# GoekeLab/m6anet

Hardware: AMD Instinct MI355X
Metric: DRACH sites/sec at num_iterations=1000 (higher is better)
Workload: dtype f32

## Files before the change

m6anet_amd/csrc/m6a_api.hip:

```cpp
#include "m6a_ctx.h"

#if !defined(__HIP_DEVICE_COMPILE__)
#ifndef M6A_MT_JUMP_PATH
#error "build with -DM6A_MT_JUMP_PATH=\"<repo>/m6anet_amd/assets/mt19937_jump.bin\" (m6anet_amd/build.py does)"
#endif
asm(".section .rodata\n"
    ".global m6a_mt_jump_blob\n.global m6a_mt_jump_blob_end\n.hidden m6a_mt_jump_blob\n.hidden m6a_mt_jump_blob_end\n.balign 64\n"
    "m6a_mt_jump_blob:\n.incbin \"" M6A_MT_JUMP_PATH "\"\n"
    "m6a_mt_jump_blob_end:\n.byte 0\n.previous\n");
#endif

namespace {

thread_local std::string g_create_error;

std::mutex g_live_mu;
std::vector<m6a_ctx *> g_live;
void join_background_setups()
{
    std::lock_guard<std::mutex> g(g_live_mu);
    for (m6a_ctx *c : g_live)
        if (c->warm.joinable()) c->warm.join();
    g_live.clear();
}
// ... 527 lines not shown
    c->bag_min = (int64_t)c->h_minmax[0];
    c->bag_max = (int64_t)c->h_minmax[1];
    c->n_reads = (int64_t)c->h_minmax[2];
    return M6A_OK;
}

int bag_stats(m6a_ctx *c, const int64_t *d_off, int64_t S)
{
    const int64_t *h = c->hint_off;
    c->hint_off = nullptr;
    if (!h) return query_bags(c, d_off, S);
    if (h[0] != 0) return fail(c, M6A_EINVAL, "off[0] must be 0");
    host_bag_range(c, h, S);
    if (c->bag_min < 0) return fail(c, M6A_EINVAL, "off[] must be non-decreasing");
    unsigned long long hash = 0;
    for (int i = 0; i < M6A_HIST_BINS; i++) hash += (unsigned long long)c->h_hist[i] * m6a_bin_weight(i);
    hipStream_t st = c->s_prep ? c->s_prep : c->stream;
    if (st != c->stream) {
        HIPCHK(c, hipEventRecord(c->ev_main, c->stream));
        HIPCHK(c, hipStreamWaitEvent(st, c->ev_main, 0));
    }
    HIPCHK(c, hipMemsetAsync(c->d_minmax, 0xff, 8, st));
    HIPCHK(c, hipMemsetAsync(c->d_minmax + 1, 0, 16, st));
    HIPCHK(c, hipMemsetAsync(c->d_hist, 0, M6A_HIST_BINS * 4, st));
    hipLaunchKernelGGL(bag_minmax_kernel, dim3((unsigned)std::min<int64_t>((S + 255) / 256, 512)), dim3(256), 0,
                       st, d_off, S, c->d_minmax, c->d_hist);
    hipLaunchKernelGGL(bag_verify_kernel, dim3(1), dim3(256), 0, st, c->d_minmax, c->d_hist, (unsigned long long)c->bag_min,
                       (unsigned long long)c->bag_max, (unsigned long long)c->n_reads, hash, c->d_err);
    HIPCHK(c, hipGetLastError());
    c->side_work = true;
    return M6A_OK;
}

static unsigned enc_args(m6a_ctx *c, EncArgs &a, const float *X, const uint8_t *km, const int64_t *off, int64_t S, int64_t R, float *rp)
{
    a.X = X; a.site_kmers = km; a.off = off; a.wfrag = c->d_wfrag; a.emb = c->d_emb; a.read_prob = rp;
    a.wfrag2 = c->d_wfrag2; a.w1e_tab = c->d_w1e; a.bn = c->d_w1e + M6A_W1E_FLOATS; a.err = c->d_err;
    a.n_sites = S; a.n_reads = R; a.n_tiles = (R + 31) / 32; a.b3 = c->b3;
    a.clk = nullptr;
    const int64_t max_waves = (int64_t)c->n_cu * 8;
    a.tiles_per_wave = (a.n_tiles + max_waves - 1) / max_waves;
    const int64_t waves = (a.n_tiles + a.tiles_per_wave - 1) / a.tiles_per_wave;
    return (unsigned)((waves + 3) / 4);
}

int launch_encode(m6a_ctx *c, const float *X, const uint8_t *km, const int64_t *off, int64_t S,
                  int64_t R, float *rp)
{
    if (R <= 0 || S <= 0) return M6A_OK;
    EncArgs a;
    const unsigned blocks = enc_args(c, a, X, km, off, S, R, rp);
    a.clk = c->prof.clk_for(0);
    const bool fits32 = S < 0x7ffffff0LL && a.n_tiles < 0x7ffffff0LL;
    if (c->enc_variant == 2 && !fits32) return fail(c, M6A_EUNSUPPORTED, "12-slot encoder: more than 2^31 sites or tiles");
    const bool scalar_chain = c->bag_min >= M6A_CSITE_MIN_BAG && fits32;
    const bool csite = c->enc_variant == 2 || (c->enc_variant == 4 && scalar_chain);
    const bool site16 = !csite && c->enc_variant != 3 && scalar_chain;
    c->enc_variant_used = csite ? "csite12" : "general16";
    c->enc_kernel_used = csite ? "enc_csite_kernel" : site16 ? "enc_site16_kernel" : "enc_kernel";
    prof_begin(c, 0);
    if (csite) hipLaunchKernelGGL(enc_csite_kernel, dim3(blocks), dim3(256), 0, c->stream, a);
    else if (site16) hipLaunchKernelGGL(enc_site16_kernel, dim3(blocks), dim3(256), 0, c->stream, a);
    else hipLaunchKernelGGL(enc_kernel, dim3(blocks), dim3(256), 0, c->stream, a);
    prof_end(c, 0);
    HIPCHK(c, hipGetLastError());
    return M6A_OK;
}

int launch_repr(m6a_ctx *c, const float *X, const uint8_t *km, const int64_t *off, int64_t S, int64_t R, void *repr, int dtype, float *rp)
{
    if (R <= 0 || S <= 0) return M6A_OK;
    EncReprArgs ra;
    const unsigned blocks = enc_args(c, ra.enc, X, km, off, S, R, rp);
    ra.repr = repr;
    c->enc_variant_used = "general16";
    c->enc_kernel_used = dtype == M6A_REPR_F16 ? "enc_repr_kernel<true>" : "enc_repr_kernel";
    prof_begin(c, 0);
    if (dtype == M6A_REPR_F16)
        hipLaunchKernelGGL(enc_repr_kernel<true>, dim3(blocks), dim3(256), 0, c->stream, ra);
    else
        hipLaunchKernelGGL(enc_repr_kernel<false>, dim3(blocks), dim3(256), 0, c->stream, ra);
    prof_end(c, 0);
    HIPCHK(c, hipGetLastError());
    return M6A_OK;
}

int repr_writer_begin(m6a_ctx *c, int device, hipStream_t *stream)
{
    settle(c);
    HintScope hint_scope(c);
    if (c->job.open) return job_busy(c);
    if (c->device != device) return fail(c, M6A_EINVAL, "the context is on device %d, the sites are on device %d", c->device, device);
    HIPCHK(c, hipSetDevice(c->device));
    *stream = c->stream;
    return M6A_OK;
}

int repr_writer_round(m6a_ctx *c, const float *X, const uint8_t *km, const int64_t *off, int64_t *off_round, int64_t s0, int64_t s1,
                      int64_t r0, int64_t nr, void *repr, int dtype)
{
    if (nr <= 0 || s1 <= s0) return M6A_OK;
    hipLaunchKernelGGL(rebase_off_kernel, dim3((unsigned)((s1 - s0 + 1 + 255) / 256)), dim3(256), 0, c->stream, off + s0, s1 - s0 + 1, off_round);
    HIPCHK(c, hipGetLastError());
    return launch_repr(c, X + r0 * 9, km + s0 * 3, off_round, s1 - s0, nr, repr, dtype, nullptr);
}

RtabUse rtab_use(m6a_ctx *c, int64_t nmax, uint32_t si_base = 0, uint32_t si_count = 0)
{
    RtabUse u;
    u.C = c->rt.C; u.RS = c->rt.RS; u.slot_of_n = (const int32_t *)c->ctl_dev.p + M6A_HIST_BINS;
    u.rank = (uint32_t *)c->rt_rank.p; u.order = (const uint32_t *)c->rt_order.p;
    u.c_stride = c->rt.n_blk * 64; u.n_blk = (uint32_t)c->rt.n_blk;
    u.bag_cap = (int)std::max<int64_t>(64, (nmax + 63) / 64 * 64);
    u.si_base = si_base; u.si_count = si_count;
    return u;
}

int rtab_prepare(m6a_ctx *c, hipStream_t st, PoolArgs a, int64_t nmax, int64_t gmax, uint32_t seed, bool *use)
{
    *use = false;
    const int T = a.T, K = a.K;
    const int64_t S = a.n_sites;
    const int64_t need = stream_need(gmax, T, K);
    if (nmax > M6A_RTAB_MAX_N || c->scan_driver == 1 || c->scan_driver == 2) {
        if (c->scan_driver == 3)
            return fail(c, M6A_EUNSUPPORTED, "index-table pooling needs every bag <= %d reads (largest: %lld)", M6A_RTAB_MAX_N, (long long)nmax);
        return M6A_OK;
    }
    int distinct = 0;
    const int missing = rtab_missing(c, seed, T, K, need, c->h_hist, &distinct);
    if (c->rt_credit_seed != seed || c->rt_credit_A != (int64_t)T * K) { c->rt_credit_seed = seed; c->rt_credit_A = (int64_t)T * K; c->rt_credit = 0; }
    bool use_rtab = c->scan_driver == 3 || missing == 0 || c->rt_credit + S >= (int64_t)16 * missing;
    if (use_rtab) c->rt_credit = 0; else c->rt_credit += S;
    if (!use_rtab) return M6A_OK;
    int rc = ensure_rtab(c, st, seed, T, K, gmax, c->h_hist, &use_rtab);
    if (rc) return rc;
    if (!use_rtab) return M6A_OK;
// ... 27 lines not shown
    unsigned blocks = 0, start_blocks = 0;
    size_t lds = 0;
    int64_t n_big = 0, cap_big = 0, cap_small = 0;
};

int pool_plan(m6a_ctx *c, hipStream_t st, const int64_t *off, int64_t S, int T, int K, uint32_t seed, int64_t bs, int64_t spb,
              PoolPlan *p)
{
    *p = PoolPlan();
    PoolArgs &a = p->a;
    if (S <= 0) return M6A_OK;
    if (c->site_mode == M6A_SITE_EXPECTED) {
        if (!base_is_group_start(c->job_offset, bs, spb))
            return fail(c, M6A_EINVAL, "job offset %lld does not start a flush group for batch_size=%lld save_per_batch=%lld",
                        (long long)c->job_offset, (long long)bs, (long long)spb);
        if (c->bag_min < 0 || c->bag_max > 0x7fffffff) return fail(c, M6A_EINVAL, "off[] is not a non-decreasing CSR array");
        a.off = off; a.n_sites = S; a.K = K;
        p->bag_min = c->bag_min; p->bag_max = c->bag_max;
        p->kind = PoolPlan::expected;
        return M6A_OK;
    }
    int rc = ensure_groups(c, st, S, bs, spb);
    if (rc) return rc;
    const int64_t nmin = c->bag_min, nmax = c->bag_max;
    if (nmin < 0 || nmax > 0x7fffffff) return fail(c, M6A_EINVAL, "off[] is not a non-decreasing CSR array");
    a.off = off; a.goff = (const int64_t *)c->goff.p; a.err = c->d_err;
    a.n_groups = c->goff_key.G; a.n_sites = S; a.T = T; a.K = K;
    const int64_t gmax = c->goff_key.gmax;

    rc = ensure_mean_plan(c, st, T);
    if (rc) return rc;
    plan_args(c, a);
    const bool uniform = nmin == nmax && nmin >= 1 && nmin <= M6A_TABLE_MAX_N && K == 20 && gmax <= 4096;
    const bool reg_ok = uniform && c->plan.depth <= M6A_REG_STACK && c->n_reads < (int64_t)1 << 30 &&
                        (int64_t)gmax * (T + 8) * K * 2 <= (int64_t)256 << 20;
    if (uniform && reg_ok && c->table_variant != 1) {
        rc = ensure_table_reg(c, st, seed, (int)nmin, T, K, (int)gmax);
        if (rc) return rc;
        a.tab = (const uint32_t *)c->tab_reg.p; a.uniform_n = (int)nmin; a.jmax = (int)gmax;
        const int64_t wpj = (a.n_groups + 255) / 256;
        a.reg_items = wpj * a.jmax;
        p->blocks = (unsigned)((a.reg_items + 7) / 8 * 8);
        p->kind = PoolPlan::table_reg;
        return M6A_OK;
    }
    if (uniform && c->plan.max_merge <= 15) {
        rc = ensure_table(c, st, seed, (int)nmin, T, K, (int)gmax);
        if (rc) return rc;
        a.tab = (const uint32_t *)c->tab.p; a.uniform_n = (int)nmin; a.jmax = (int)gmax;
        const int64_t gblocks = (a.n_groups + 7) / 8;
        int64_t nbj = std::max<int64_t>(1, ((int64_t)c->n_cu * 5 + a.jmax - 1) / a.jmax);
        nbj = std::min<int64_t>(nbj, (gblocks + 3) / 4);
        p->blocks = (unsigned)(nbj * a.jmax);
        p->lds = (size_t)4 * (128 + 8 * a.stack_depth) * sizeof(float);
        p->kind = PoolPlan::table;
        return M6A_OK;
    }
    bool use_rtab = false;
    rc = rtab_prepare(c, st, a, nmax, gmax, seed, &use_rtab);
    if (rc) return rc;
    if (use_rtab) {
        a.raw = (const uint32_t *)c->raw.p; a.raw_len = c->raw_len;
        for (int n = M6A_RTAB_SMALL_N + 1; n < M6A_HIST_BINS; n++) p->n_big += c->h_hist[n];
        p->cap_big = nmax; p->cap_small = std::min<int64_t>(nmax, M6A_RTAB_SMALL_N);
        p->kind = PoolPlan::ragged_table;
        return M6A_OK;
    }
// ... 492 lines not shown
        rc = bag_stats(c, off, S);
        if (rc) return rc;
        return launch_repr(c, X, km, off, S, c->n_reads, repr, dtype, rp);
    }
    rc = csr_check(c, off, S);
    if (rc) return rc;
    const int64_t R = off[S];
    if (R == 0) return M6A_OK;
    const int64_t chunk_reads = (int64_t)1 << 20;
    std::vector<int64_t> cs{0};
    int64_t widest = 0;
    while (cs.back() < S) {
        const int64_t s0 = cs.back();
        int64_t s1 = std::upper_bound(off + s0, off + S + 1, off[s0] + chunk_reads) - off - 1;
        s1 = std::min<int64_t>(S, std::max<int64_t>(s1, s0 + 1));
        widest = std::max(widest, off[s1] - off[s0]);
        cs.push_back(s1);
    }
    const int64_t nchunk = (int64_t)cs.size() - 1;
    HIPCHK(c, c->sX.ensure((size_t)widest * 9 * 4));
    HIPCHK(c, c->sOffChunk.ensure((size_t)(S + nchunk) * 8));
    HIPCHK(c, c->sRepr.ensure((size_t)widest * row_bytes));
    if (rp) HIPCHK(c, c->sP.ensure((size_t)widest * 4));
    HIPCHK(c, stage_in(c, c->sK, km, (size_t)S * 3));
    HIPCHK(c, stage_in(c, c->sOff, off, (size_t)(S + 1) * 8));
    for (int64_t k = 0; k < nchunk; k++) {
        const int64_t s0 = cs[k], s1 = cs[k + 1], r0 = off[s0], nr = off[s1] - r0;
        if (nr == 0) continue;
        HIPCHK(c, hipMemcpyAsync(c->sX.p, X + r0 * 9, (size_t)nr * 9 * 4, hipMemcpyHostToDevice, c->stream));
        int64_t *d_off = (int64_t *)c->sOffChunk.p + s0 + k;
        hipLaunchKernelGGL(rebase_off_kernel, dim3((unsigned)((s1 - s0 + 1 + 255) / 256)), dim3(256), 0, c->stream,
                           (const int64_t *)c->sOff.p + s0, s1 - s0 + 1, d_off);
        rc = launch_repr(c, (const float *)c->sX.p, (const uint8_t *)c->sK.p + s0 * 3, d_off, s1 - s0, nr, c->sRepr.p, dtype,
                         rp ? (float *)c->sP.p : nullptr);
        if (rc) return rc;
        HIPCHK(c, stage_out(c, (char *)repr + (size_t)r0 * row_bytes, c->sRepr, (size_t)nr * row_bytes));
        if (rp) HIPCHK(c, stage_out(c, rp + r0, c->sP, (size_t)nr * 4));
        HIPCHK(c, hipStreamSynchronize(c->stream));
    }
    return sync_and_check(c);
}

static int pool_stage_in(m6a_ctx *c, const float *rp, const int64_t *off, int64_t S, bool sigma)
{
    int rc = csr_check(c, off, S);
    if (rc) return rc;
    HIPCHK(c, c->sSite.ensure((size_t)S * 4));
    HIPCHK(c, c->sMod.ensure((size_t)S * 8));
    if (sigma) HIPCHK(c, c->sSigma.ensure((size_t)S * 8));
    HIPCHK(c, stage_in(c, c->sP, rp, (size_t)off[S] * 4));
    HIPCHK(c, stage_in(c, c->sOff, off, (size_t)(S + 1) * 8));
    host_bag_range(c, off, S);
    return M6A_OK;
}

static int pool_stage_out(m6a_ctx *c, int64_t S, float *site, double *mod, double *sigma)
{
    HIPCHK(c, stage_out(c, site, c->sSite, (size_t)S * 4));
    HIPCHK(c, stage_out(c, mod, c->sMod, (size_t)S * 8));
    if (sigma) HIPCHK(c, stage_out(c, sigma, c->sSigma, (size_t)S * 8));
    return sync_and_check(c);
}

int m6a_site_pool(m6a_ctx *c, const float *rp, const int64_t *off, int64_t S, int T, int K, float thr,
                  uint32_t seed, int rng_mode, int64_t bs, int64_t spb, float *site, double *mod)
{
    HintScope hint_scope(c);
// ... 279 lines not shown
```

m6anet_amd/csrc/m6a_ctx.h:

```cpp
#pragma once
#include <hip/hip_runtime.h>
#include <dlfcn.h>
#include <sys/mman.h>

#include <algorithm>
#include <atomic>
#include <cmath>
#include <cstdarg>
#include <cstdio>
#include <cstdlib>
#include <cstring>
#include <condition_variable>
#include <functional>
#include <memory>
#include <mutex>
#include <new>
#include <string>
#include <thread>
#include <vector>

#include "m6a.h"
#include "m6a_kernels.h"
#include "m6a_host_cpus.h"

// ... 256 lines not shown

static inline int enter(m6a_ctx *c)
{
    settle(c);
    if (!c) return M6A_EINVAL;
    return job_busy(c);
}

static inline int same_side(m6a_ctx *c, const void *first, std::initializer_list<const void *> rest, const char *sentence)
{
    const bool dev = is_device_ptr(first);
    for (const void *p : rest)
        if (p && dev != is_device_ptr(p)) return fail(c, M6A_EINVAL, "%s", sentence);
    return dev;
}

static inline int csr_check(m6a_ctx *c, const int64_t *off, int64_t S)
{
    if (off[0] != 0) return fail(c, M6A_EINVAL, "off[0] must be 0");
    for (int64_t s = 0; s < S; s++) if (off[s + 1] < off[s]) return fail(c, M6A_EINVAL, "off[] must be non-decreasing");
    return M6A_OK;
}

static inline hipError_t stage_in(m6a_ctx *c, DevBuf &b, const void *host, size_t bytes)
{
    const hipError_t e = b.ensure(bytes ? bytes : 1);
    return e != hipSuccess ? e : hipMemcpyAsync(b.p, host, bytes, hipMemcpyHostToDevice, c->stream);
}
static inline hipError_t stage_out(m6a_ctx *c, void *host, const DevBuf &b, size_t bytes)
{
    return hipMemcpyAsync(host, b.p, bytes, hipMemcpyDeviceToHost, c->stream);
}

int launch_encode(m6a_ctx *c, const float *X, const uint8_t *km, const int64_t *off, int64_t S, int64_t R, float *rp);
int launch_repr(m6a_ctx *c, const float *X, const uint8_t *km, const int64_t *off, int64_t S, int64_t R, void *repr, int dtype, float *rp);
int repr_writer_begin(m6a_ctx *c, int device, hipStream_t *stream);
int repr_writer_round(m6a_ctx *c, const float *X, const uint8_t *km, const int64_t *off, int64_t *off_round, int64_t s0, int64_t s1,
                      int64_t r0, int64_t nr, void *repr, int dtype);
int launch_pool(m6a_ctx *c, const float *rp, const int64_t *off, int64_t S, int T, int K, float thr, uint32_t seed, int64_t bs, int64_t spb,
                float *site, double *mod);
int bag_stats(m6a_ctx *c, const int64_t *d_off, int64_t S);
void host_bag_range(m6a_ctx *c, const int64_t *off, int64_t S);
void prof_begin(m6a_ctx *c, int kind);
void prof_end(m6a_ctx *c, int kind);
int ensure_staging(m6a_ctx *c);
void release_staging(m6a_ctx *c);
int staged_encode(m6a_ctx *c, const float *X, const uint8_t *km, const int64_t *off, int64_t S, int64_t R, float *rp_host);
int staged_outputs(m6a_ctx *c, int64_t S, float *site, double *mod);
int d2h_through_ring(m6a_ctx *c, void *host, const void *dev, size_t bytes);
bool base_is_group_start(int64_t base, int64_t bs, int64_t spb);
void comm_release(m6a_ctx *c);

}
```

m6anet_amd/csrc/m6a_job.hip:

```cpp
#include "m6a_ctx.h"

using namespace m6a_detail;

namespace m6a_detail {

int grow_keep(m6a_ctx *c, DevBuf &b, size_t used_bytes, size_t need_bytes)
{
    if (need_bytes <= b.cap) return M6A_OK;
    const size_t want = std::max(need_bytes + need_bytes / 8 + 256, b.cap * 2);
    void *np_ = nullptr;
    HIPCHK(c, hipMalloc(&np_, want));
    if (b.p && used_bytes) {
        if (c->stg.s_h2d) HIPCHK(c, hipStreamSynchronize(c->stg.s_h2d));
        HIPCHK(c, hipMemcpyAsync(np_, b.p, used_bytes, hipMemcpyDeviceToDevice, c->stream));
        HIPCHK(c, hipStreamSynchronize(c->stream));
    }
    if (b.p) (void)hipFree(b.p);
    b.p = np_; b.cap = want;
    return M6A_OK;
}

int job_setup_ring(m6a_ctx *c)
{
    auto &j = c->job;
// ... 36 lines not shown
    if (!j.cur_ready) {
        if (j.used[(size_t)sub]) HIPCHK(c, hipEventSynchronize(j.ev_h2d[(size_t)sub]));
        j.cur_ready = true;
    }
    *pin = j.pin[(size_t)sub];
    return M6A_OK;
}

int job_flush(m6a_ctx *c, const float *dX = nullptr, const uint8_t *dK = nullptr)
{
    auto &j = c->job;
    Staging &g = c->stg;
    if (j.fill_sites == 0) return M6A_OK;
    const int sub = (int)(j.item % j.n_sub);
    char *pin = j.pin[(size_t)sub];
    char *dev = (char *)c->jX.p + (size_t)sub * j.sub_bytes;
    const int64_t ns = j.fill_sites, nr = j.fill_reads, s0 = j.S - ns, r0 = j.R - nr;
    int rc = grow_keep(c, c->jP, (size_t)r0 * 4, (size_t)std::max<int64_t>(j.R, 1) * 4);
    if (rc) return rc;
    rc = grow_keep(c, c->jOff, (size_t)(s0 + 1) * 8, (size_t)(j.S + 1) * 8);
    if (rc) return rc;
    if (j.used[(size_t)sub]) HIPCHK(c, hipStreamWaitEvent(g.s_h2d, j.ev_enc[(size_t)sub], 0));
    HIPCHK(c, hipMemcpyAsync(dev, pin, (size_t)(ns + 1) * 8, hipMemcpyHostToDevice, g.s_h2d));
    HIPCHK(c, hipMemcpyAsync((int64_t *)c->jOff.p + s0, pin + j.o_goff, (size_t)(ns + 1) * 8, hipMemcpyHostToDevice, g.s_h2d));
    if (!dX) {
        HIPCHK(c, hipMemcpyAsync(dev + j.o_km, pin + j.o_km, (size_t)ns * 3, hipMemcpyHostToDevice, g.s_h2d));
        if (nr) HIPCHK(c, hipMemcpyAsync(dev + j.o_x, pin + j.o_x, (size_t)nr * M6A_N_FEATURES * 4, hipMemcpyHostToDevice, g.s_h2d));
    }
    HIPCHK(c, hipEventRecord(j.ev_h2d[(size_t)sub], g.s_h2d));
    HIPCHK(c, hipStreamWaitEvent(c->stream, j.ev_h2d[(size_t)sub], 0));
    if (nr) {
        c->bag_min = j.fill_min; c->n_reads = nr;
        rc = launch_encode(c, dX ? dX : (const float *)(dev + j.o_x), dK ? dK : (const uint8_t *)(dev + j.o_km), (const int64_t *)dev, ns, nr,
                           (float *)c->jP.p + r0);
        if (rc) return rc;
    }
    HIPCHK(c, hipEventRecord(j.ev_enc[(size_t)sub], c->stream));
    j.used[(size_t)sub] = 1;
    j.item++; j.chunks++;
    j.fill_sites = 0; j.fill_reads = 0; j.fill_min = INT64_MAX; j.cur_ready = false;
    return M6A_OK;
}

void job_append_offsets(m6a_ctx *c, char *pin, const int64_t *off, int64_t i, int64_t k)
{
    auto &j = c->job;
    int64_t *ol = (int64_t *)pin, *og = (int64_t *)(pin + j.o_goff);
    if (j.fill_sites == 0) { ol[0] = 0; og[0] = j.R; }
    const int64_t base = off[i], lbase = j.fill_reads, gbase = j.R;
    int64_t mn = j.fill_min;
    for (int64_t t = 0; t < k; t++) {
        const int64_t e = off[i + t + 1] - base, n = off[i + t + 1] - off[i + t];
        ol[j.fill_sites + t + 1] = lbase + e;
        og[j.fill_sites + t + 1] = gbase + e;
        j.off.push_back(gbase + e);
        mn = n < mn ? n : mn;
    }
    j.fill_min = mn;
    const int64_t nr = off[i + k] - base;
    j.fill_sites += k; j.fill_reads += nr; j.S += k; j.R += nr;
}

int job_feed_impl(m6a_ctx *c, const float *X, const uint8_t *km, const int64_t *off, int64_t n, bool dev)
{
    auto &j = c->job;
    int rc = csr_check(c, off, n);
    if (rc) return rc;
// ... 213 lines not shown
```

m6anet_amd/csrc/m6a_kernels.h:

```cpp
#ifndef M6A_KERNELS_H
#define M6A_KERNELS_H
#include <hip/hip_runtime.h>
#include <stdint.h>

#define M6A_BAG_LDS 1024
#define M6A_WFRAG_FLOATS (136 * 64)
#define M6A_WFRAG2_FLOATS (25 * 64)
#define M6A_W1E_FLOATS (35 * 32)
#define M6A_BN_FLOATS (5 * 2 * 16 * 2)
#define M6A_MEAN_STACK 32
#define M6A_CSITE_MIN_BAG 16
#define M6A_TABLE_MAX_N 32
#define M6A_REG_STACK 8
#define M6A_RTAB_MAX_N 4096
#define M6A_RTAB_SMALL_N 1024
#define M6A_RTAB_U8_MAX_N 256
#define M6A_HIST_BINS (M6A_RTAB_MAX_N + 2)

__host__ __device__ inline unsigned long long m6a_bin_weight(int i)
{
    unsigned long long z = (unsigned long long)(i + 1) * 0x9E3779B97F4A7C15ull;
    z = (z ^ (z >> 30)) * 0xBF58476D1CE4E5B9ull;
    z = (z ^ (z >> 27)) * 0x94D049BB133111EBull;
    return z ^ (z >> 31);
}

#define M6A_CLK_SLOTS 64
__device__ __forceinline__ void m6a_clk_stamp(unsigned long long *clk, int which)
{
    if (!clk) return;
    const unsigned stride = (gridDim.x >> 6) | 1u, b = blockIdx.x;
    if (threadIdx.x == 0 && b % stride == 0 && b / stride < M6A_CLK_SLOTS) {
        unsigned long long *p = clk + (size_t)(b / stride) * 4 + which * 2;
        p[0] = __builtin_amdgcn_s_memtime();
        p[1] = __builtin_amdgcn_s_memrealtime();
    }
}

struct EncArgs {
    const float *X;
    const uint8_t *site_kmers;
    const int64_t *off;
    const float *wfrag;
    const float *wfrag2;
    const float *w1e_tab;
    const float *bn;
    const float *emb;
    float *read_prob;
    int *err;
    int64_t n_sites, n_reads, n_tiles, tiles_per_wave;
    float b3;
    unsigned long long *clk;
};

struct EncReprArgs {
    EncArgs enc;
    void *repr;
};

struct PoolArgs {
    const float *read_prob;
    const int64_t *off;
    const int64_t *goff;
    const uint32_t *raw;
    const uint32_t *tab;
    float *site_prob;
    double *mod_ratio;
    uint32_t *start_pos;
    const int *leaf_start;
    const uint8_t *merge_after;
    const uint32_t *row_meta;
    int n_leaves, n_rows, n_rem;
    int stack_depth;
    const uint32_t *reg_ctl;
    int reg_rounds, reg_final_merges;
    int64_t reg_items;
    int *err;
    int64_t n_groups, n_sites, raw_len;
    int T, K, uniform_n, jmax, bag_cap;
    float thr;
    unsigned long long *clk;
};

// ... 70 lines not shown
```

m6anet_amd/csrc/m6a_kernels.hip:

```cpp
#include <hip/hip_runtime.h>
#include <stdint.h>

#include "m6a_kernels.h"

typedef float f32x16 __attribute__((ext_vector_type(16)));
typedef float f32x2 __attribute__((ext_vector_type(2)));

__device__ __forceinline__ float chain8_sum(float r)
{
    r += __builtin_bit_cast(float, __builtin_amdgcn_update_dpp(0, __builtin_bit_cast(int, r), 0xB1, 0xf, 0xf, false));
    r += __builtin_bit_cast(float, __builtin_amdgcn_update_dpp(0, __builtin_bit_cast(int, r), 0x4E, 0xf, 0xf, false));
    r += __builtin_bit_cast(float, __builtin_amdgcn_update_dpp(0, __builtin_bit_cast(int, r), 0x141, 0xf, 0xf, false));
    return r;
}

__device__ __forceinline__ int wave_sum_i32(int v)
{
#pragma unroll
    for (int m = 1; m < 64; m <<= 1) v += __shfl_xor(v, m, 64);
    return v;
}

#define L2_REGS(m) ((m) == 4 ? 12 : 16)

// ... 99 lines not shown
{
    return ((int64_t)__builtin_amdgcn_readfirstlane((int)(v >> 32)) << 32) |
           (uint32_t)__builtin_amdgcn_readfirstlane((int)v);
}

__device__ __forceinline__ void wave_lds_fence()
{
    __builtin_amdgcn_fence(__ATOMIC_ACQ_REL, "wavefront");
    __builtin_amdgcn_wave_barrier();
}

struct EncLds {
    float emb[132];
    __attribute__((aligned(16))) float bn[M6A_BN_FLOATS];
};
__device__ __forceinline__ void stage_lds(EncLds &s, const EncArgs &a)
{
    for (int i = threadIdx.x; i < 132; i += 256) s.emb[i] = a.emb[i];
    for (int i = threadIdx.x; i < M6A_BN_FLOATS; i += 256) s.bn[i] = a.bn[i];
}

template <int N> __device__ __forceinline__ void load_frag(float (&w)[N], const float *frag, int lane)
{
#pragma unroll
    for (int i = 0; i < N; i++) w[i] = frag[i * 64 + lane];
}
__device__ __forceinline__ void load_frags16(const float *wfrag, int lane, float (&w1)[40], float (&w2)[80], float (&w3)[16])
{
    load_frag(w1, wfrag, lane);
    load_frag(w2, wfrag + 40 * 64, lane);
    load_frag(w3, wfrag + 120 * 64, lane);
}

template <typename I> __device__ __forceinline__ I first_site(const int64_t *off, I n_sites, int64_t r)
{
    I lo = 0, hi = n_sites;
    while (hi - lo > 1) {
        const I mid = (I)(((int64_t)lo + hi) >> 1);
        if (off[mid] <= r) lo = mid; else hi = mid;
    }
    return lo;
}

__device__ __forceinline__ void layer1_16(int m, f32x16 &acc, const float (&w1)[40], const float (&f)[8])
{
#pragma unroll
    for (int q = 0; q < 16; q++) acc[q] = 0.0f;
#pragma unroll
    for (int st = 0; st < 8; st++)
        acc = __builtin_amdgcn_mfma_f32_32x32x2f32(w1[m * 8 + st], f[st], acc, 0, 0, 0);
}

template <class Layer1, class Links>
__device__ __forceinline__ void unit_tile_loop(f32x16 &acc2, const float (&w2)[80], BnPairs &bnq, const float *bn_half, Layer1 &&layer1, Links &&links)
{
    f32x16 h1a, h1b;
#pragma unroll
    for (int q = 0; q < 16; q++) acc2[q] = 0.0f;
    layer1(0, h1a);
#pragma unroll
    for (int m = 0; m < 5; m++) {
        f32x16 &cur = (m & 1) ? h1b : h1a;
        f32x16 &nxt = (m & 1) ? h1a : h1b;
        if (m < 4) layer1(m + 1, nxt);
        __builtin_amdgcn_sched_barrier(0);
        links(m);
        if (m == 0) layer2_with_bn<0>(acc2, cur, w2, bnq, bn_half);
        if (m == 1) layer2_with_bn<1>(acc2, cur, w2, bnq, bn_half);
        if (m == 2) layer2_with_bn<2>(acc2, cur, w2, bnq, bn_half);
// ... 43 lines not shown
            w[j].w = f16_pair(v[2 * j + 1].z, v[2 * j + 1].w);
        }
        if (mine) {
            uint4 *dst = (uint4 *)((uint16_t *)repr + r * 32 + half * 16);
            dst[0] = w[0];
            dst[1] = w[1];
        }
    } else if (mine) {
        float4 *dst = (float4 *)((float *)repr + r * 32 + half * 16);
#pragma unroll
        for (int j = 0; j < 4; j++) dst[j] = v[j];
    }
}

enum { REPR_NONE, REPR_F32, REPR_F16 };
template <int REPR> __device__ __forceinline__ void enc_walk_tiles(const EncArgs &a, void *repr)
{
    __shared__ EncLds lds;
    stage_lds(lds, a);
    __syncthreads();

    const int lane = threadIdx.x & 63;
    const int col = lane & 31;
    const int half = lane >> 5;
    const float *bn_half = lds.bn + half * 32;
    const int64_t wave = (int64_t)blockIdx.x * 4 + __builtin_amdgcn_readfirstlane((int)(threadIdx.x >> 6));
    const int64_t tile0 = wave * a.tiles_per_wave;
    if (tile0 >= a.n_tiles) return;
    const int64_t tile1 = (tile0 + a.tiles_per_wave < a.n_tiles) ? tile0 + a.tiles_per_wave : a.n_tiles;

    float w1[40], w2[80], w3[16];
    load_frags16(a.wfrag, lane, w1, w2, w3);

    int64_t s_base = first_site<int64_t>(a.off, a.n_sites, tile0 * 32);
    const int64_t last_site = a.n_sites - 1;

    auto link0 = [&](int64_t base, int64_t (&o)[3]) {
#pragma unroll
        for (int i = 0; i < 3; i++) {
            const int64_t si = base + 1 + i;
            o[i] = a.off[si <= a.n_sites ? si : a.n_sites];
        }
    };
    auto link1 = [&](int64_t tile, int64_t base, const int64_t (&o)[3], int64_t &s, int (&km)[3], float (&x)[8]) {
        const int64_t r = tile * 32 + col;
        const int64_t rc = r < a.n_reads ? r : a.n_reads - 1;
        s = base + (rc >= o[0] ? 1 : 0) + (rc >= o[1] ? 1 : 0);
        if (__any(rc >= o[2])) {
            s = base;
            while (a.off[s + 1] <= rc) ++s;
        }
        s = s < last_site ? s : last_site;
        const uint8_t *kp = a.site_kmers + s * 3;
        km[0] = kp[0]; km[1] = kp[1]; km[2] = kp[2];
        const float *xp = a.X + rc * 9 + half;
#pragma unroll
        for (int i = 0; i < 4; i++) x[i] = xp[2 * i];
        x[4] = xp[half ? 6 : 8];
    };
    auto link2 = [&](const int (&km)[3], float (&x)[8]) {
        const float e0 = lds.emb[2 * km[0] + 1 - half], e1 = lds.emb[2 * km[1] + 1 - half], e2 = lds.emb[2 * km[2] + 1 - half];
        x[4] = half ? e0 : x[4];
        x[5] = half ? e1 : e0;
        x[6] = half ? e2 : e1;
        x[7] = half ? 1.0f : e2;
    };

// ... 48 lines not shown
}
template __global__ void enc_repr_kernel<false>(EncReprArgs ra);
template __global__ void enc_repr_kernel<true>(EncReprArgs ra);

struct ScalarChain {
    const EncArgs &a;
    const float *s_emb;
    const __attribute__((address_space(4))) int64_t *off_c;
    int lane, col, half, wave;
    int n_tiles, tile0, tile1, n_sites, last_site;
    int last_lim;
    int kq_site, kq_byte;
    int too_small = 0;

    __device__ __forceinline__ ScalarChain(const EncArgs &args, const float *emb)
        : a(args), s_emb(emb), off_c((const __attribute__((address_space(4))) int64_t *)args.off)
    {
        lane = threadIdx.x & 63;
        col = lane & 31;
        half = lane >> 5;
        wave = (int)blockIdx.x * 4 + __builtin_amdgcn_readfirstlane((int)(threadIdx.x >> 6));
        n_tiles = (int)a.n_tiles;
        const int tpw = (int)a.tiles_per_wave;
        tile0 = wave * tpw;
        tile1 = (tile0 + tpw < n_tiles) ? tile0 + tpw : n_tiles;
        n_sites = (int)a.n_sites;
        last_site = n_sites - 1;
        last_lim = (int)(a.n_reads - 1 - (int64_t)(n_tiles - 1) * 32);
        const int kq = lane < 18 ? lane : 17;
        kq_site = kq / 6;
        kq_byte = (kq % 6) / 2;
    }
    __device__ __forceinline__ int lim(int tile) const { return tile == n_tiles - 1 ? last_lim : 31; }
    __device__ __forceinline__ int start() const { return __builtin_amdgcn_readfirstlane(first_site<int>(a.off, n_sites, (int64_t)tile0 * 32)); }
    __device__ __forceinline__ void link0(int base, int64_t (&o)[3]) const
    {
#pragma unroll
        for (int i = 0; i < 3; i++) {
            const int si = base + 1 + i;
            o[i] = off_c[si <= n_sites ? si : n_sites];
        }
    }
    template <int N> __device__ __forceinline__ void link1(int tile, int base, const int64_t (&o)[3], int &rel, int &kid, float (&x)[N])
    {
        const int64_t rbase = (int64_t)tile * 32;
        const int crel = col < lim(tile) ? col : lim(tile);
        const int d0 = (int)o[0] - (int)rbase, d1 = (int)o[1] - (int)rbase, d2 = (int)o[2] - (int)rbase;
        rel = (crel >= d0 ? 1 : 0) + (crel >= d1 ? 1 : 0);
        too_small |= lim(tile) >= d2 ? 1 : 0;
        const int room = last_site - base;
        const int ksr = kq_site < room ? kq_site : room;
        kid = (int)(a.site_kmers + (int64_t)base * 3)[__umul24((unsigned)ksr, 3u) + (unsigned)kq_byte];
        const float *xt = a.X + rbase * 9;
        const float *xp = (const float *)((const char *)xt + (unsigned)(4 * (crel * 9 + half)));
#pragma unroll
        for (int i = 0; i < 4; i++) x[i] = xp[2 * i];
        x[4] = *(const float *)((const char *)xt + (unsigned)(4 * (crel * 9 + (half ? 7 : 8))));
    }
    __device__ __forceinline__ void link2(int kid, float &ev) const { ev = s_emb[2 * kid + (lane & 1)]; }
    __device__ __forceinline__ int advance(int rel) const { return __builtin_amdgcn_readfirstlane(__shfl(rel, 31, 64)); }
    __device__ __forceinline__ void raise_too_small() const
    {
        if (too_small && lane == 0) atomicExch(a.err, 2);
    }
};

__global__ __launch_bounds__(256, 2) void enc_site16_kernel(EncArgs a)
// ... 832 lines not shown
```

m6anet_amd/csrc/m6a_pool_reg.hip:

```cpp
#include "m6a_kernels.h"

#define S1(x) #x
#define S(x) S1(x)

#define MUL0 \
    "v_pk_mul_f32 v[56:57], v[128:129], 1.0 op_sel_hi:[1,0]\n" \
    "v_pk_mul_f32 v[58:59], v[192:193], 1.0 op_sel_hi:[1,0]\n"
#define MUL \
    "v_pk_mul_f32 v[56:57], v[128:129], v[56:57]\n" \
    "v_pk_mul_f32 v[58:59], v[192:193], v[58:59]\n"
#define LO(r) "s_sext_i32_i16 m0, s[" S(r) "]\n"
#define HI(r) "s_lshr_b32 m0, s[" S(r) "], 16\n"
#define DRAW2(r) LO(r) MUL HI(r) MUL
#define DRAWS(b) \
    "s_set_gpr_idx_on s[" S(b) "], gpr_idx(SRC0)\n" \
    MUL0 HI(b) MUL \
    DRAW2(b+1) DRAW2(b+2) DRAW2(b+3) DRAW2(b+4) DRAW2(b+5) DRAW2(b+6) DRAW2(b+7) DRAW2(b+8) DRAW2(b+9) \
    "s_set_gpr_idx_off\n" \
    "v_pk_add_f32 v[56:57], v[56:57], 1.0 op_sel_hi:[1,0] neg_lo:[1,0] neg_hi:[1,0]\n" \
    "v_pk_add_f32 v[58:59], v[58:59], 1.0 op_sel_hi:[1,0] neg_lo:[1,0] neg_hi:[1,0]\n"

#define ITER(i, b) \
    DRAWS(b) \
    "v_pk_add_f32 v[96+4*" S(i) ":97+4*" S(i) "], v[96+4*" S(i) ":97+4*" S(i) "], v[56:57]\n" \
// ... 23 lines not shown
#define MERGES(lbl) \
    "s_cmp_eq_u32 s79, 0\n" \
    "s_cbranch_scc1 " lbl "f\n" \
    lbl "0:\n" \
    "s_sub_u32 s78, s78, 4\n" \
    "s_set_gpr_idx_on s78, gpr_idx(SRC0)\n" \
    "v_pk_add_f32 v[60:61], v[64:65], v[60:61]\n" \
    "v_pk_add_f32 v[62:63], v[66:67], v[62:63]\n" \
    "s_set_gpr_idx_off\n" \
    "s_sub_u32 s79, s79, 1\n" \
    "s_cmp_lg_u32 s79, 0\n" \
    "s_cbranch_scc1 " lbl "0b\n" \
    lbl ":\n"

__global__ __launch_bounds__(64) void pool_reg_kernel(PoolArgs a)
{
    const int lane = threadIdx.x;
    const unsigned per = gridDim.x >> 3;
    const unsigned item = (blockIdx.x & 7u) * per + (blockIdx.x >> 3);
    if (item >= (unsigned)a.reg_items) return;
    m6a_clk_stamp(a.clk, 0);
    const int j = (int)(item % (unsigned)a.jmax);
    const int64_t g0 = (int64_t)(item / (unsigned)a.jmax) * 256;
    int64_t site[4];
    uint32_t boff[4];
#pragma unroll
    for (int q = 0; q < 4; q++) {
        const int64_t g = g0 + q * 64 + lane;
        site[q] = -1;
        if (g < a.n_groups) {
            const int64_t s = a.goff[g] + j;
            if (s < a.goff[g + 1]) site[q] = s;
        }
        boff[q] = site[q] >= 0 ? (uint32_t)(a.off[site[q]] * 4) : 0u;
    }
    const uint64_t rp = (uint64_t)a.read_prob;
    const uint64_t tab = (uint64_t)((const uint8_t *)a.tab + (size_t)j * (size_t)(a.T + 8) * 40);
    const uint64_t ctl = (uint64_t)a.reg_ctl;
    float o0, o1, o2, o3;
    int c0, c1, c2, c3;
    asm volatile(
        "v_mov_b32 v32, %[b0]\n"
        "v_mov_b32 v33, %[b1]\n"
        "v_mov_b32 v34, %[b2]\n"
        "v_mov_b32 v35, %[b3]\n"
        "s_mov_b64 s[80:81], %[tab]\n"
        "s_mov_b64 s[82:83], %[ctl]\n"
        "s_load_dwordx16 s[36:51], s[80:81], 0\n"
        "s_load_dwordx4 s[52:55], s[80:81], 64\n"
        "s_load_dwordx16 s[56:71], s[80:81], 80\n"
        "s_load_dwordx4 s[72:75], s[80:81], 144\n"
        "s_mov_b32 s77, %[nr]\n"
        "s_mov_b32 s78, 0\n"
        "v_mov_b32 v40, 0\n"
        "v_mov_b32 v41, 0\n"
        "v_mov_b32 v42, 0\n"
        "v_mov_b32 v43, 0\n"
        "s_and_b32 s79, %[n], 3\n"
        "s_cmp_eq_u32 s79, 0\n"
        "s_cbranch_scc0 80f\n"
        "s_lshr_b32 s79, %[n], 2\n"
        ".set m6a_e, 0\n"
        ".rept 8\n"
        "s_cmp_lt_u32 m6a_e, s79\n"
        "s_cbranch_scc0 81f\n"
        "global_load_dwordx4 v[64+4*m6a_e:67+4*m6a_e], v32, %[rp] offset:16*m6a_e\n"
        "global_load_dwordx4 v[96+4*m6a_e:99+4*m6a_e], v33, %[rp] offset:16*m6a_e\n"
        "global_load_dwordx4 v[128+4*m6a_e:131+4*m6a_e], v34, %[rp] offset:16*m6a_e\n"
        "global_load_dwordx4 v[160+4*m6a_e:163+4*m6a_e], v35, %[rp] offset:16*m6a_e\n"
        ".set m6a_e, m6a_e+1\n"
        ".endr\n"
        "81:\n"
        "s_waitcnt vmcnt(0)\n"
        ".set m6a_e, 0\n"
        ".rept 32\n"
        "s_cmp_lt_u32 m6a_e, %[n]\n"
        "s_cselect_b64 s[84:85], exec, 0\n"
        "v_cmp_le_f32 vcc, %[thr], v[64+m6a_e]\n"
        "s_and_b64 vcc, vcc, s[84:85]\n"
        "v_addc_co_u32 v40, vcc, 0, v40, vcc\n"
        "v_cmp_le_f32 vcc, %[thr], v[96+m6a_e]\n"
        "s_and_b64 vcc, vcc, s[84:85]\n"
        "v_addc_co_u32 v41, vcc, 0, v41, vcc\n"
        "v_cmp_le_f32 vcc, %[thr], v[128+m6a_e]\n"
        "s_and_b64 vcc, vcc, s[84:85]\n"
        "v_addc_co_u32 v42, vcc, 0, v42, vcc\n"
        "v_cmp_le_f32 vcc, %[thr], v[160+m6a_e]\n"
        "s_and_b64 vcc, vcc, s[84:85]\n"
        "v_addc_co_u32 v43, vcc, 0, v43, vcc\n"
        ".set m6a_e, m6a_e+1\n"
        ".endr\n"
        ".set m6a_e, 0\n"
        ".rept 32\n"
        "v_sub_f32 v[192+2*m6a_e], 1.0, v[128+m6a_e]\n"
        "v_sub_f32 v[193+2*m6a_e], 1.0, v[160+m6a_e]\n"
        ".set m6a_e, m6a_e+1\n"
        ".endr\n"
        ".set m6a_e, 0\n"
        ".rept 32\n"
        "v_sub_f32 v[128+2*m6a_e], 1.0, v[64+m6a_e]\n"
        "v_sub_f32 v[129+2*m6a_e], 1.0, v[96+m6a_e]\n"
        ".set m6a_e, m6a_e+1\n"
        ".endr\n"
        ".set m6a_i, 0\n"
        ".rept 64\n"
        "v_mov_b32 v[64+m6a_i], 0\n"
        ".set m6a_i, m6a_i+1\n"
        ".endr\n"
        "s_branch 82f\n"
        "80:\n"
        "s_sub_u32 s79, %[n], 1\n"
        ".set m6a_e, 0\n"
        ".rept 32\n"
        "global_load_dword v[128+2*m6a_e], v32, %[rp]\n"
        "s_cmp_lt_u32 m6a_e, s79\n"
        "s_cselect_b32 s76, 4, 0\n"
        "v_add_u32 v32, s76, v32\n"
        ".set m6a_e, m6a_e+1\n"
        ".endr\n"
        ".set m6a_e, 0\n"
        ".rept 32\n"
        "global_load_dword v[129+2*m6a_e], v33, %[rp]\n"
        "s_cmp_lt_u32 m6a_e, s79\n"
        "s_cselect_b32 s76, 4, 0\n"
        "v_add_u32 v33, s76, v33\n"
        ".set m6a_e, m6a_e+1\n"
        ".endr\n"
        ".set m6a_e, 0\n"
        ".rept 32\n"
        "global_load_dword v[192+2*m6a_e], v34, %[rp]\n"
        "s_cmp_lt_u32 m6a_e, s79\n"
        "s_cselect_b32 s76, 4, 0\n"
        "v_add_u32 v34, s76, v34\n"
        ".set m6a_e, m6a_e+1\n"
        ".endr\n"
        ".set m6a_e, 0\n"
// ... 143 lines not shown
```

Measured before the change: 386.6 million.

## Narrow encoder site search with bag bounds and skip unused pool-reg slots

The encoder's first_site binary search now uses the known min/max bag sizes to narrow the search window before bisecting. It falls back to the full range when bounds are unknown, such as in job and repr-writer paths. The register pooling kernel computes read offsets directly from site*uniform_n instead of loading off[], with a new guard requiring n_reads == S*nmin. Its unrolled compare/subtract loops also branch out in blocks of four once past n, skipping dead work for small bags. The risks are wrong narrowing if the bag bounds are stale, and added branch overhead.

```diff
diff --git a/m6anet_amd/csrc/m6a_api.hip b/m6anet_amd/csrc/m6a_api.hip
--- a/m6anet_amd/csrc/m6a_api.hip
+++ b/m6anet_amd/csrc/m6a_api.hip
@@ -583,11 +583,13 @@
     return M6A_OK;
 }
 
-static unsigned enc_args(m6a_ctx *c, EncArgs &a, const float *X, const uint8_t *km, const int64_t *off, int64_t S, int64_t R, float *rp)
+static unsigned enc_args(m6a_ctx *c, EncArgs &a, const float *X, const uint8_t *km, const int64_t *off, int64_t S, int64_t R, float *rp,
+                         bool bags_known = true)
 {
     a.X = X; a.site_kmers = km; a.off = off; a.wfrag = c->d_wfrag; a.emb = c->d_emb; a.read_prob = rp;
     a.wfrag2 = c->d_wfrag2; a.w1e_tab = c->d_w1e; a.bn = c->d_w1e + M6A_W1E_FLOATS; a.err = c->d_err;
     a.n_sites = S; a.n_reads = R; a.n_tiles = (R + 31) / 32; a.b3 = c->b3;
+    a.bag_min = bags_known ? c->bag_min : 0; a.bag_max = bags_known ? c->bag_max : 0;
     a.clk = nullptr;
     const int64_t max_waves = (int64_t)c->n_cu * 8;
     a.tiles_per_wave = (a.n_tiles + max_waves - 1) / max_waves;
@@ -596,11 +598,11 @@
 }
 
 int launch_encode(m6a_ctx *c, const float *X, const uint8_t *km, const int64_t *off, int64_t S,
-                  int64_t R, float *rp)
+                  int64_t R, float *rp, bool bags_known)
 {
     if (R <= 0 || S <= 0) return M6A_OK;
     EncArgs a;
-    const unsigned blocks = enc_args(c, a, X, km, off, S, R, rp);
+    const unsigned blocks = enc_args(c, a, X, km, off, S, R, rp, bags_known);
     a.clk = c->prof.clk_for(0);
     const bool fits32 = S < 0x7ffffff0LL && a.n_tiles < 0x7ffffff0LL;
     if (c->enc_variant == 2 && !fits32) return fail(c, M6A_EUNSUPPORTED, "12-slot encoder: more than 2^31 sites or tiles");
@@ -618,11 +620,12 @@
     return M6A_OK;
 }
 
-int launch_repr(m6a_ctx *c, const float *X, const uint8_t *km, const int64_t *off, int64_t S, int64_t R, void *repr, int dtype, float *rp)
+int launch_repr(m6a_ctx *c, const float *X, const uint8_t *km, const int64_t *off, int64_t S, int64_t R, void *repr, int dtype, float *rp,
+                bool bags_known)
 {
     if (R <= 0 || S <= 0) return M6A_OK;
     EncReprArgs ra;
-    const unsigned blocks = enc_args(c, ra.enc, X, km, off, S, R, rp);
+    const unsigned blocks = enc_args(c, ra.enc, X, km, off, S, R, rp, bags_known);
     ra.repr = repr;
     c->enc_variant_used = "general16";
     c->enc_kernel_used = dtype == M6A_REPR_F16 ? "enc_repr_kernel<true>" : "enc_repr_kernel";
@@ -653,7 +656,7 @@
     if (nr <= 0 || s1 <= s0) return M6A_OK;
     hipLaunchKernelGGL(rebase_off_kernel, dim3((unsigned)((s1 - s0 + 1 + 255) / 256)), dim3(256), 0, c->stream, off + s0, s1 - s0 + 1, off_round);
     HIPCHK(c, hipGetLastError());
-    return launch_repr(c, X + r0 * 9, km + s0 * 3, off_round, s1 - s0, nr, repr, dtype, nullptr);
+    return launch_repr(c, X + r0 * 9, km + s0 * 3, off_round, s1 - s0, nr, repr, dtype, nullptr, false);
 }
 
 RtabUse rtab_use(m6a_ctx *c, int64_t nmax, uint32_t si_base = 0, uint32_t si_count = 0)
@@ -747,7 +750,7 @@
     if (rc) return rc;
     plan_args(c, a);
     const bool uniform = nmin == nmax && nmin >= 1 && nmin <= M6A_TABLE_MAX_N && K == 20 && gmax <= 4096;
-    const bool reg_ok = uniform && c->plan.depth <= M6A_REG_STACK && c->n_reads < (int64_t)1 << 30 &&
+    const bool reg_ok = uniform && c->plan.depth <= M6A_REG_STACK && c->n_reads < (int64_t)1 << 30 && c->n_reads == S * nmin &&
                         (int64_t)gmax * (T + 8) * K * 2 <= (int64_t)256 << 20;
     if (uniform && reg_ok && c->table_variant != 1) {
         rc = ensure_table_reg(c, st, seed, (int)nmin, T, K, (int)gmax);
@@ -1306,7 +1309,7 @@
         hipLaunchKernelGGL(rebase_off_kernel, dim3((unsigned)((s1 - s0 + 1 + 255) / 256)), dim3(256), 0, c->stream,
                            (const int64_t *)c->sOff.p + s0, s1 - s0 + 1, d_off);
         rc = launch_repr(c, (const float *)c->sX.p, (const uint8_t *)c->sK.p + s0 * 3, d_off, s1 - s0, nr, c->sRepr.p, dtype,
-                         rp ? (float *)c->sP.p : nullptr);
+                         rp ? (float *)c->sP.p : nullptr, false);
         if (rc) return rc;
         HIPCHK(c, stage_out(c, (char *)repr + (size_t)r0 * row_bytes, c->sRepr, (size_t)nr * row_bytes));
         if (rp) HIPCHK(c, stage_out(c, rp + r0, c->sP, (size_t)nr * 4));
diff --git a/m6anet_amd/csrc/m6a_ctx.h b/m6anet_amd/csrc/m6a_ctx.h
--- a/m6anet_amd/csrc/m6a_ctx.h
+++ b/m6anet_amd/csrc/m6a_ctx.h
@@ -312,8 +312,9 @@
     return hipMemcpyAsync(host, b.p, bytes, hipMemcpyDeviceToHost, c->stream);
 }
 
-int launch_encode(m6a_ctx *c, const float *X, const uint8_t *km, const int64_t *off, int64_t S, int64_t R, float *rp);
-int launch_repr(m6a_ctx *c, const float *X, const uint8_t *km, const int64_t *off, int64_t S, int64_t R, void *repr, int dtype, float *rp);
+int launch_encode(m6a_ctx *c, const float *X, const uint8_t *km, const int64_t *off, int64_t S, int64_t R, float *rp, bool bags_known = true);
+int launch_repr(m6a_ctx *c, const float *X, const uint8_t *km, const int64_t *off, int64_t S, int64_t R, void *repr, int dtype, float *rp,
+                bool bags_known = true);
 int repr_writer_begin(m6a_ctx *c, int device, hipStream_t *stream);
 int repr_writer_round(m6a_ctx *c, const float *X, const uint8_t *km, const int64_t *off, int64_t *off_round, int64_t s0, int64_t s1,
                       int64_t r0, int64_t nr, void *repr, int dtype);
diff --git a/m6anet_amd/csrc/m6a_job.hip b/m6anet_amd/csrc/m6a_job.hip
--- a/m6anet_amd/csrc/m6a_job.hip
+++ b/m6anet_amd/csrc/m6a_job.hip
@@ -92,7 +92,7 @@
     if (nr) {
         c->bag_min = j.fill_min; c->n_reads = nr;
         rc = launch_encode(c, dX ? dX : (const float *)(dev + j.o_x), dK ? dK : (const uint8_t *)(dev + j.o_km), (const int64_t *)dev, ns, nr,
-                           (float *)c->jP.p + r0);
+                           (float *)c->jP.p + r0, false);
         if (rc) return rc;
     }
     HIPCHK(c, hipEventRecord(j.ev_enc[(size_t)sub], c->stream));
diff --git a/m6anet_amd/csrc/m6a_kernels.h b/m6anet_amd/csrc/m6a_kernels.h
--- a/m6anet_amd/csrc/m6a_kernels.h
+++ b/m6anet_amd/csrc/m6a_kernels.h
@@ -49,6 +49,7 @@
     float *read_prob;
     int *err;
     int64_t n_sites, n_reads, n_tiles, tiles_per_wave;
+    int64_t bag_min, bag_max;
     float b3;
     unsigned long long *clk;
 };
diff --git a/m6anet_amd/csrc/m6a_kernels.hip b/m6anet_amd/csrc/m6a_kernels.hip
--- a/m6anet_amd/csrc/m6a_kernels.hip
+++ b/m6anet_amd/csrc/m6a_kernels.hip
@@ -155,9 +155,16 @@
     load_frag(w3, wfrag + 120 * 64, lane);
 }
 
-template <typename I> __device__ __forceinline__ I first_site(const int64_t *off, I n_sites, int64_t r)
-{
-    I lo = 0, hi = n_sites;
+template <typename I, typename P> __device__ __forceinline__ I first_site(P off, I n_sites, int64_t r, int64_t bag_min, int64_t bag_max)
+{
+    const bool usable = bag_min > 0 && bag_max >= bag_min;
+    const double rd = (double)r;
+    const uint64_t first = (uint64_t)(rd / (double)(usable ? bag_max : 1)), last = (uint64_t)(rd / (double)(usable ? bag_min : 1));
+    const uint64_t top = (uint64_t)n_sites - 1;
+    const I blo = (I)(first < top ? first : top), bhi = (I)(last < top ? last + 1 : top + 1);
+    const int64_t olo = off[blo], ohi = off[bhi];
+    const bool narrowed = usable && first <= top && olo <= r && r < ohi;
+    I lo = narrowed ? blo : 0, hi = narrowed ? bhi : n_sites;
     while (hi - lo > 1) {
         const I mid = (I)(((int64_t)lo + hi) >> 1);
         if (off[mid] <= r) lo = mid; else hi = mid;
@@ -267,7 +274,7 @@
     float w1[40], w2[80], w3[16];
     load_frags16(a.wfrag, lane, w1, w2, w3);
 
-    int64_t s_base = first_site<int64_t>(a.off, a.n_sites, tile0 * 32);
+    int64_t s_base = first_site<int64_t>(a.off, a.n_sites, tile0 * 32, a.bag_min, a.bag_max);
     const int64_t last_site = a.n_sites - 1;
 
     auto link0 = [&](int64_t base, int64_t (&o)[3]) {
@@ -382,7 +389,10 @@
         kq_byte = (kq % 6) / 2;
     }
     __device__ __forceinline__ int lim(int tile) const { return tile == n_tiles - 1 ? last_lim : 31; }
-    __device__ __forceinline__ int start() const { return __builtin_amdgcn_readfirstlane(first_site<int>(a.off, n_sites, (int64_t)tile0 * 32)); }
+    __device__ __forceinline__ int start() const
+    {
+        return __builtin_amdgcn_readfirstlane(first_site<int>(off_c, n_sites, (int64_t)tile0 * 32, a.bag_min, a.bag_max));
+    }
     __device__ __forceinline__ void link0(int base, int64_t (&o)[3]) const
     {
 #pragma unroll
diff --git a/m6anet_amd/csrc/m6a_pool_reg.hip b/m6anet_amd/csrc/m6a_pool_reg.hip
--- a/m6anet_amd/csrc/m6a_pool_reg.hip
+++ b/m6anet_amd/csrc/m6a_pool_reg.hip
@@ -79,7 +79,7 @@
             const int64_t s = a.goff[g] + j;
             if (s < a.goff[g + 1]) site[q] = s;
         }
-        boff[q] = site[q] >= 0 ? (uint32_t)(a.off[site[q]] * 4) : 0u;
+        boff[q] = site[q] >= 0 ? (uint32_t)site[q] * (uint32_t)a.uniform_n * 4u : 0u;
     }
     const uint64_t rp = (uint64_t)a.read_prob;
     const uint64_t tab = (uint64_t)((const uint8_t *)a.tab + (size_t)j * (size_t)(a.T + 8) * 40);
@@ -120,35 +120,44 @@
         "81:\n"
         "s_waitcnt vmcnt(0)\n"
         ".set m6a_e, 0\n"
-        ".rept 32\n"
+        ".rept 8\n"
         "s_cmp_lt_u32 m6a_e, %[n]\n"
-        "s_cselect_b64 s[84:85], exec, 0\n"
+        "s_cbranch_scc0 83f\n"
+        ".rept 4\n"
         "v_cmp_le_f32 vcc, %[thr], v[64+m6a_e]\n"
-        "s_and_b64 vcc, vcc, s[84:85]\n"
         "v_addc_co_u32 v40, vcc, 0, v40, vcc\n"
         "v_cmp_le_f32 vcc, %[thr], v[96+m6a_e]\n"
-        "s_and_b64 vcc, vcc, s[84:85]\n"
         "v_addc_co_u32 v41, vcc, 0, v41, vcc\n"
         "v_cmp_le_f32 vcc, %[thr], v[128+m6a_e]\n"
-        "s_and_b64 vcc, vcc, s[84:85]\n"
         "v_addc_co_u32 v42, vcc, 0, v42, vcc\n"
         "v_cmp_le_f32 vcc, %[thr], v[160+m6a_e]\n"
-        "s_and_b64 vcc, vcc, s[84:85]\n"
         "v_addc_co_u32 v43, vcc, 0, v43, vcc\n"
         ".set m6a_e, m6a_e+1\n"
         ".endr\n"
-        ".set m6a_e, 0\n"
-        ".rept 32\n"
+        ".endr\n"
+        "83:\n"
+        ".set m6a_e, 0\n"
+        ".rept 8\n"
+        "s_cmp_lt_u32 m6a_e, %[n]\n"
+        "s_cbranch_scc0 84f\n"
+        ".rept 4\n"
         "v_sub_f32 v[192+2*m6a_e], 1.0, v[128+m6a_e]\n"
         "v_sub_f32 v[193+2*m6a_e], 1.0, v[160+m6a_e]\n"
         ".set m6a_e, m6a_e+1\n"
         ".endr\n"
-        ".set m6a_e, 0\n"
-        ".rept 32\n"
+        ".endr\n"
+        "84:\n"
+        ".set m6a_e, 0\n"
+        ".rept 8\n"
+        "s_cmp_lt_u32 m6a_e, %[n]\n"
+        "s_cbranch_scc0 85f\n"
+        ".rept 4\n"
         "v_sub_f32 v[128+2*m6a_e], 1.0, v[64+m6a_e]\n"
         "v_sub_f32 v[129+2*m6a_e], 1.0, v[96+m6a_e]\n"
         ".set m6a_e, m6a_e+1\n"
         ".endr\n"
+        ".endr\n"
+        "85:\n"
         ".set m6a_i, 0\n"
         ".rept 64\n"
         "v_mov_b32 v[64+m6a_i], 0\n"
```

Result: no change. 388.8 million (median of 6 runs) (+0.6%).
